# vdBerg93/cl-rrt

Hardware: AMD Instinct MI355X
Metric: nodes expanded/sec (200-obstacle scene) (higher is better)
Workload: dtype f64

## Files before the change

### cl-rrt_amd/csrc/clrrt_capi.hip

```cpp
#include <hip/hip_runtime.h>
#include <math.h>

#include <algorithm>
#include <climits>
#include <array>
#include <chrono>
#include <cmath>
#include <cstdio>
#include <cstdlib>
#include <cstring>
#include <deque>
#include <functional>
#include <optional>
#include <string>
#include <vector>

#include "../../include/clrrt.h"
#include "clrrt_dev.hpp"
#include "clrrt_internal.hpp"

static const int kWalkMaxOver = 2048, kWalkMaxChunks = 64;

using namespace clrrt;

// ... 146 lines not shown
  hipStream_t side2 = nullptr;
  hipStream_t mst = nullptr;
  int nn_delta_walk = 1;
  int nn_delta_verify = 0;
  WalkBufs nnw_d{};
  WalkBufs nnw_r{};
  struct {
    int64_t n = -1, first = 0, count = 0;
    double ox, oy, x0, y0, x1, y1;
    float delta;
    int kind, hscale;
  } nnr_built;
  int* pm_ids = nullptr;
  float* pm_keys = nullptr;
  int* pm_counts = nullptr;
  int64_t pm_cap = 0;
  int* d_bad = nullptr;
  float* vpk = nullptr;
  int* vpi = nullptr;
  float* vseed = nullptr;
  int nn_delta_early = 1;
  int nn_lane_order = 1;
  int* nn_order = nullptr;
  float* wseed[3] = {nullptr, nullptr, nullptr};
  hipEvent_t ev_wm[3] = {nullptr, nullptr, nullptr};
  hipEvent_t ev_lagw[3] = {nullptr, nullptr, nullptr};
  int stream_prio = 1;
  int walk_cu_reserve = 0;
  hipEvent_t ev_lag[3] = {nullptr, nullptr, nullptr};
  int stream_prio_applied = 0;
  bool side_prio_set = false;
  std::vector<clrrt_sample> pf_next, pf_samples;
  int pf_state = 0;
  struct {
    int T = 0;
    bool active = false;
    int R = 0;
    int T_alloc = 0, n_steps_alloc = 0;
    int64_t vcap = 0;
    RollRes* res = nullptr;
    RollRes* res_gb = nullptr;
    int* cand = nullptr;
    int* ncand = nullptr;
    clrrt_sample* samp = nullptr;
    int* best = nullptr;
    int* dlist[2] = {nullptr, nullptr};
    int cur_dl = 0, nd = 0;
    int nd_eval = -1;
    int* gv = nullptr;
    uint8_t* pend = nullptr;
    void* sel_tmp = nullptr;
    size_t sel_bytes = 0;
    int* d_cnt = nullptr;
    void* carry[2] = {nullptr, nullptr};
    int cur_c = 0, ncarry = 0, carry_cap = 0;
    int64_t round = 0;
    int slot = 0;
    int64_t deferred_total = 0;
  } def;
  struct {
    int rank = 0, world = 1;
    void* dev_local = nullptr;
    int cap_local = 0;
    clrrt_exchange_fn fn = nullptr;
    void* user = nullptr;
    double max_ms = 0;
    int64_t nd_global = 0;
    int64_t rows_stop = 0;
    int last_nb = 0;
    clrrt_node* xbuf = nullptr;
    uint32_t* xkey = nullptr;
    void* xtmp = nullptr;
    size_t xtmp_bytes = 0;
    int64_t xcap = 0;
    unsigned long long* d_goal = nullptr;
    bool poison_seen = false;
    bool fn_failed = false;
    bool hook_world1 = false;
  } sh;
  int fail_at_round = 0;
  int fail_after_exchange = 0;
  bool debug_sync = false;
  unsigned long long* dbg_host = nullptr;
  bool iter_log = false;
  std::vector<int64_t> round_sizes;
  std::vector<clrrt_iteration> iters;
  std::vector<SampleOut> iter_tmp;
  clrrt_sample* h_samples = nullptr;
  int64_t* h_totals = nullptr;
  int* h_int = nullptr;
  int64_t last_eval_rows = 0;
  int64_t last_goal_nodes = 0;
  clrrt_counters counters{};
  int64_t nn_bf_keys = 0, nn_samples = 0;
  int64_t nn_super_bounds = 0;
  bool timing = false;
  static constexpr int kKtClasses = 6;
  double kt_ms[kKtClasses] = {};
  int64_t kt_n[kKtClasses] = {};
  std::vector<hipEvent_t> ev_pool;
  std::vector<std::pair<int, std::pair<hipEvent_t, hipEvent_t>>> ev_pending;
};

static void pf_reset(clrrt_ctx* c);
static int flush_replays(clrrt_ctx* c);
static int append_nodes(clrrt_ctx* c, const clrrt_node* dev_nodes, int n);
static int watchdog_check(clrrt_ctx* c);
static void defer_roll_args(clrrt_ctx* c, RollArgs& a, bool capped);
static int commit_round(clrrt_ctx* c, int nn, double elapsed_ms, int* n_app);
static int ensure_slots(clrrt_ctx* c);

static int fail(clrrt_ctx* c, int code, const std::string& msg) {
  if (c) c->err = msg;
  return code;
}
#define HIPC(c, call)                                                                          \
  do {                                                                                         \
    hipError_t e_ = (call);                                                                    \
    if (e_ != hipSuccess)                                                                      \
      return fail((c), CLRRT_EHIP, std::string(#call) + ": " + hipGetErrorString(e_));        \
  } while (0)

template <typename T>
static hipError_t dalloc(T** p, size_t count) {
  *p = nullptr;
  if (count == 0) count = 1;
  return hipMalloc((void**)p, count * sizeof(T));
}

static hipEvent_t ev_get(clrrt_ctx* c) {
  if (!c->ev_pool.empty()) {
    hipEvent_t e = c->ev_pool.back();
    c->ev_pool.pop_back();
    return e;
  }
  hipEvent_t e;
  if (hipEventCreate(&e) != hipSuccess) return nullptr;
  return e;
}

struct KTimer {
  clrrt_ctx* c;
  int which;
  hipEvent_t a = nullptr, b = nullptr;
  hipStream_t s;
  KTimer(clrrt_ctx* c_, int w, hipStream_t s_ = nullptr) : c(c_), which(w), s(s_ ? s_ : c_->stream) {
    if (!c->timing) return;
    a = ev_get(c);
    b = ev_get(c);
    if (a) hipEventRecord(a, s);
  }
  ~KTimer() {
    if (!c->timing || !a || !b) return;
    hipEventRecord(b, s);
    c->ev_pending.push_back({which, {a, b}});
  }
};

static void drain_timers(clrrt_ctx* c) {
  for (auto& pe : c->ev_pending) {
    float ms = 0;
    hipEventSynchronize(pe.second.second);
    if (hipEventElapsedTime(&ms, pe.second.first, pe.second.second) == hipSuccess) {
      c->kt_ms[pe.first] += ms;
      c->kt_n[pe.first] += 1;
    }
// ... 149 lines not shown
static void free_all(clrrt_ctx* c) {
  if (c->side) hipStreamSynchronize(c->side);
  void* ptrs[] = {c->tree, c->nn, c->arena, c->obs, c->d_samples, c->pk, c->pi, c->cand, c->ckey, c->ncand,
                  c->ctie, c->sort_scratch, c->res_spec, c->regnodes, c->res_gb, c->gbnodes, c->so, c->first_conflict,
                  c->out_nodes, c->jobs, c->slots, c->rep_buf, c->totals, c->work_ctr, c->grid_buf,
                  c->nn_seed, c->d_bbox, c->roll_q, c->roll_best, c->roll_perm, c->roll_pflag,
                  c->goal_recs, c->bp_path, c->path_nodes, c->path_rows, c->ri_int, c->ri_off, c->ri_cost,
                  c->ri_terms, c->nnw.keys, c->nnw.keys2, c->nnw.vals, c->nnw.vals2, c->nnw.tmp, c->nnw.P, c->nnw.Q,
                  c->nnw.CE, c->nnw.ID, c->nnw.tiles, c->nnw.supers, c->nnw.sorder, c->nnw.HEAD, c->nnw.ovf_n, c->nnw.ovf, c->nnw.pk, c->nnw.pi, c->nnw_alt.keys, c->nnw_alt.keys2, c->nnw_alt.vals, c->nnw_alt.vals2, c->nnw_alt.tmp, c->nnw_alt.P, c->nnw_alt.Q, c->nnw_alt.CE, c->nnw_alt.ID, c->nnw_alt.tiles, c->nnw_alt.supers, c->nnw_alt.sorder, c->nnw_alt.HEAD, c->nnw_alt.ovf_n, c->nnw_alt.ovf, c->nnw_alt.pk, c->nnw_alt.pi, c->nnw.skeys, c->nnw.sids, c->nnw_alt.skeys, c->nnw_alt.sids, c->cmp.packed, c->cmp.scanned,
                  c->cmp.tmp, c->d_samples2, c->cand2, c->ckey2, c->ncand2, c->ctie2, c->d_samples3, c->cand3, c->ckey3,
                  c->ncand3, c->ctie3, c->nnw3.keys, c->nnw3.keys2, c->nnw3.vals, c->nnw3.vals2, c->nnw3.tmp, c->nnw3.P,
                  c->nnw3.Q, c->nnw3.CE, c->nnw3.ID, c->nnw3.tiles, c->nnw3.supers, c->nnw3.sorder, c->nnw3.HEAD,
                  c->nnw3.ovf_n, c->nnw3.ovf, c->nnw3.pk, c->nnw3.pi, c->nnw3.skeys, c->nnw3.sids,
                  c->nnw.trun, c->nnw_alt.trun, c->nnw3.trun, c->nnw.wctr, c->nnw_alt.wctr, c->nnw3.wctr};
  for (void* p : ptrs)
    if (p) hipFree(p);
  void* sptrs[] = {c->sh.xbuf, c->sh.xkey, c->sh.xtmp, c->sh.d_goal, c->fix_n, c->fix_ids, c->fix_jobs, c->fix_res, c->fix_adj,
                   c->fix_xrec, c->fix_xi, c->fix_xcand, c->fix_xkey, c->fix_xn};
  for (void* p : sptrs)
    if (p) hipFree(p);
  void* dptrs[] = {c->def.res, c->def.res_gb, c->def.cand, c->def.ncand, c->def.samp, c->def.best, c->def.dlist[0],
                   c->def.dlist[1], c->def.gv, c->def.pend, c->def.sel_tmp, c->def.d_cnt, c->def.carry[0],
                   c->def.carry[1]};
  for (void* p : dptrs)
    if (p) hipFree(p);
  if (c->h_samples) hipHostFree(c->h_samples);
  if (c->h_samples2) hipHostFree(c->h_samples2);
  if (c->h_samples3) hipHostFree(c->h_samples3);
  if (c->side2) hipStreamSynchronize(c->side2);
  if (c->side2) hipStreamDestroy(c->side2);
  for (auto e : c->ev_lag)
    if (e) hipEventDestroy(e);
  for (auto e : c->ev_lagw)
    if (e) hipEventDestroy(e);
  if (c->mst) hipStreamSynchronize(c->mst);
  if (c->mst) hipStreamDestroy(c->mst);
  for (int q = 0; q < 3; q++) {
    if (c->wseed[q]) hipFree(c->wseed[q]);
    if (q == 0 && c->nn_order) hipFree(c->nn_order);
    if (c->ev_wm[q]) hipEventDestroy(c->ev_wm[q]);
  }
  {
    WalkBufs& d = c->nnw_d;
    void* wd[] = {d.keys, d.vals, d.tmp, d.P, d.Q, d.CE, d.ID, d.HEAD, d.trun, d.tiles, d.supers, d.skeys, d.sids,
                  c->vpk, c->vpi, c->vseed};
    for (void* p : wd)
      if (p) hipFree(p);
  }
  {
    WalkBufs& r = c->nnw_r;
    void* wr[] = {r.keys, r.keys2, r.vals, r.vals2, r.tmp, r.P, r.Q, r.CE, r.ID, r.tiles, r.supers, r.sorder, r.HEAD,
                  r.ovf_n, r.ovf, r.pk, r.pi, r.skeys, r.sids, r.trun, r.wctr, c->pm_ids, c->pm_keys, c->pm_counts,
                  c->d_bad};
    for (void* p : wr)
      if (p) hipFree(p);
  }
  if (c->side) hipStreamSynchronize(c->side);
  if (c->ev_tree) hipEventDestroy(c->ev_tree);
  if (c->ev_walk) hipEventDestroy(c->ev_walk);
  if (c->ev_commit) hipEventDestroy(c->ev_commit);
  if (c->side) hipStreamDestroy(c->side);
  if (c->roll_st) hipStreamDestroy(c->roll_st);
  if (c->ev_rs0) hipEventDestroy(c->ev_rs0);
  if (c->ev_rs1) hipEventDestroy(c->ev_rs1);
  if (c->h_totals) hipHostFree(c->h_totals);
  if (c->h_int) hipHostFree(c->h_int);
  if (c->h_bbox) hipHostFree(c->h_bbox);
  if (c->dbg_host) hipHostFree(c->dbg_host);
  for (auto& pe : c->ev_pending) { hipEventDestroy(pe.second.first); hipEventDestroy(pe.second.second); }
  for (auto e : c->ev_pool) hipEventDestroy(e);
  if (c->own_stream && c->stream) hipStreamDestroy(c->stream);
}

int clrrt_create(const clrrt_params* p, const clrrt_capacity* cap, int device, clrrt_ctx** out) {
  if (!p || !out) return CLRRT_EINVAL;
  *out = nullptr;
  int ndev = 0;
  if (hipGetDeviceCount(&ndev) != hipSuccess || ndev <= 0) return CLRRT_EHIP;
  if (device < 0 || device >= ndev) return CLRRT_EINVAL;
  clrrt_ctx* c = new clrrt_ctx();
  c->device = device;
  c->params = *p;
  c->debug_sync = getenv("CLRRT_DEBUG_SYNC") != nullptr;
  clrrt_capacity dc;
  dc.max_nodes = 1 << 20;
  dc.max_rows = 1 << 24;
  dc.max_batch = 4096;
  dc.max_obstacles = 4096;
  c->cap = cap ? *cap : dc;
  if (c->cap.max_nodes < 2 || c->cap.max_rows < 2 || c->cap.max_batch < 1 || c->cap.max_obstacles < 0) {
    delete c;
    return CLRRT_EINVAL;
  }
  derive(c->params, c->dp, 0);
  int rc = CLRRT_OK;
  auto chk = [&](hipError_t e) {
    if (e != hipSuccess && rc == CLRRT_OK) { rc = CLRRT_EHIP; c->err = hipGetErrorString(e); }
  };
  chk(hipSetDevice(device));
  chk(hipStreamCreateWithFlags(&c->stream, hipStreamNonBlocking));
  c->own_stream = true;
  const int64_t B = c->cap.max_batch;
  chk(dalloc(&c->tree, c->cap.max_nodes));
  chk(dalloc(&c->nn, c->cap.max_nodes));
  chk(dalloc(&c->arena, (size_t)c->cap.max_rows * 10));
  chk(dalloc(&c->obs, std::max<int64_t>(1, c->cap.max_obstacles)));
  chk(dalloc(&c->d_samples, B));
  c->partial_cap = std::max<int64_t>(B * 16, 4096) * NN_K;
  chk(dalloc(&c->pk, c->partial_cap));
  chk(dalloc(&c->pi, c->partial_cap));
  chk(dalloc(&c->cand, B * CAND_K));
  chk(dalloc(&c->ckey, B * CAND_K));
  chk(dalloc(&c->ncand, B));
  chk(dalloc(&c->ctie, B));
  chk(dalloc(&c->d_samples2, B));
  chk(dalloc(&c->cand2, B * CAND_K));
  chk(dalloc(&c->ckey2, B * CAND_K));
  chk(dalloc(&c->ncand2, B));
  chk(dalloc(&c->ctie2, B));
  chk(hipStreamCreateWithFlags(&c->side, hipStreamNonBlocking));
  chk(hipEventCreateWithFlags(&c->ev_tree, hipEventDisableTiming));
  chk(hipEventCreateWithFlags(&c->ev_walk, hipEventDisableTiming));
  chk(hipEventCreateWithFlags(&c->ev_commit, hipEventDisableTiming));
  chk(dalloc(&c->res_spec, B * CAND_K));
  chk(dalloc(&c->regnodes, B));
  chk(dalloc(&c->res_gb, B * CAND_K));
  c->slot_rows = 0;
  chk(hipMalloc(&c->rep_buf, replay_bytes() * (size_t)2 * B));
  chk(dalloc(&c->gbnodes, B));
  chk(dalloc(&c->so, B));
  chk(dalloc(&c->first_conflict, 1));
  chk(dalloc(&c->out_nodes, 2 * B));
  chk(dalloc(&c->jobs, 2 * B));
  chk(dalloc(&c->totals, 8));
  chk(dalloc(&c->cmp.packed, B));
  chk(dalloc(&c->cmp.scanned, B));
  c->cmp.tmp_bytes = compact_scan_bytes((int)B);
  chk(hipMalloc(&c->cmp.tmp, std::max<size_t>(c->cmp.tmp_bytes, 256)));
  chk(dalloc(&c->nn_seed, B));
  chk(dalloc(&c->roll_q, 1));
  chk(dalloc(&c->roll_best, B));
  chk(dalloc(&c->roll_perm, (int64_t)B * CAND_K));
  chk(dalloc(&c->roll_pflag, (int64_t)roll_order_ints((int)(B * CAND_K))));
  {
    int ncu = 0;
    if (hipDeviceGetAttribute(&ncu, hipDeviceAttributeMultiprocessorCount, device) == hipSuccess && ncu > 0)
      c->n_cu = ncu;
  }
  chk(dalloc(&c->d_bbox, 4));
  chk(hipHostMalloc((void**)&c->h_bbox, sizeof(double) * 4, hipHostMallocDefault));
  chk(dalloc(&c->work_ctr, 64));
  if (rc == CLRRT_OK) chk(hipMemset(c->work_ctr, 0, 64 * sizeof(unsigned long long)));
  chk(hipHostMalloc((void**)&c->h_samples, sizeof(clrrt_sample) * B, hipHostMallocDefault));
  chk(hipHostMalloc((void**)&c->h_samples2, sizeof(clrrt_sample) * B, hipHostMallocDefault));
  chk(hipHostMalloc((void**)&c->h_totals, sizeof(int64_t) * 8, hipHostMallocDefault));
  chk(hipHostMalloc((void**)&c->h_int, sizeof(int) * 4, hipHostMallocDefault));
  if (rc != CLRRT_OK) {
    fprintf(stderr, "clrrt_create: %s\n", c->err.c_str());
    free_all(c);
    delete c;
    return rc;
  }
  *out = c;
  return CLRRT_OK;
}

// ... 1217 lines not shown
    if (rc != CLRRT_OK) return rc;
  }
  if (pre_roll) {
    int rc = pre_roll();
    if (rc != CLRRT_OK) return rc;
  }
  if (during_roll) HIPC(c, hipEventRecord(c->ev_tree, st));
  hipStream_t rst = st;
  if (c->roll_st) {
    rst = c->roll_st;
    HIPC(c, hipEventRecord(c->ev_rs0, st));
    HIPC(c, hipStreamWaitEvent(rst, c->ev_rs0, 0));
  }
  const bool persistent = c->roll_persistent && c->dp.n_steps_max > 0;
  const bool deferred = persistent && c->rows_deferred;
  if (!deferred) {
    int rc = flush_replays(c);
    if (rc == CLRRT_OK) rc = ensure_slots(c);
    if (rc != CLRRT_OK) return rc;
  }
  const bool defer = c->def.active && !exact && persistent && deferred;
  if (defer) {
    auto& d = c->def;
    d.slot = (int)(d.round % d.R);
    const int64_t B = c->cap.max_batch;
    HIPC(c, hipMemcpyAsync(d.cand + (int64_t)d.slot * B * CAND_K, c->cand, sizeof(int) * n * CAND_K,
                           hipMemcpyDeviceToDevice, st));
    HIPC(c, hipMemcpyAsync(d.ncand + (int64_t)d.slot * B, c->ncand, sizeof(int) * n, hipMemcpyDeviceToDevice, st));
    HIPC(c, hipMemcpyAsync(d.samp + (int64_t)d.slot * B, c->d_samples, sizeof(clrrt_sample) * n,
                           hipMemcpyDeviceToDevice, st));
    if (d.nd + (int64_t)n > d.vcap) return fail(c, CLRRT_ECAPACITY, "deferred samples exceed the commit buffers");
    if (rst != st) {
      HIPC(c, hipEventRecord(c->ev_rs0, st));
      HIPC(c, hipStreamWaitEvent(rst, c->ev_rs0, 0));
    }
  }
  {
    KTimer kt(c, 1, rst);
    RollArgs a = roll_args(c, n * CAND_K);
    a.res = c->res_spec;
    a.res_gb = c->res_gb;
    if (defer) defer_roll_args(c, a, true);
    a.slots = deferred ? nullptr : c->slots;
    a.slot_rows = c->slot_rows;
    a.slot_jobs = (int)(c->cap.max_batch * CAND_K);
    if (deferred) {
      a.rep = c->rep_buf;
      a.nrep = c->rep_n;
    }
    const int64_t nt = c->n_nodes;
    const int eighths = nt < 300000 ? 7 : nt < 700000 ? 5 : nt < 1100000 ? 4 : 2;
    const int blocks = c->roll_blocks > 0 ? std::min(c->roll_blocks, 4 * c->n_cu)
                       : c->cu_split > 0  ? std::max(1, (c->cu_split * c->n_cu) / 8)
                                          : std::max(1, (eighths * c->n_cu) / 8);
    a.coop_enable = c->roll_coop;
    a.lanes_per_wave = c->roll_lanes > 0 ? c->roll_lanes : c->roll_spread ? 0 : 64;
    if (c->roll_priority) {
      a.perm = c->roll_perm;
      a.pflag = c->roll_pflag;
      a.order_verify = c->roll_order_verify;
    }
    unsigned long long*& dbg_host = c->dbg_host;
    if (c->debug_sync) {
      if (!dbg_host) HIPC(c, hipHostMalloc((void**)&dbg_host, sizeof(unsigned long long) * 8 * 4096, hipHostMallocMapped));
      memset(dbg_host, 0, sizeof(unsigned long long) * 8 * 4096);
      HIPC(c, hipHostGetDevicePointer((void**)&a.dbg, dbg_host, 0));
      HIPC(c, hipStreamSynchronize(rst));
      fprintf(stderr, "[dbg] pre-rollout work done (n %d, nrep %d, ncarry %d)\n", n, a.nrep, a.ncarry);
    }
    if (persistent && defer) {
      FillInts f;
      f.add(a.ncarry_out, 1, 0);
      f.add(c->roll_q, 1, 0);
      f.add(c->def.best + a.sbase, n, 0x7f7f7f7f);
      f.add(c->def.d_cnt + 2, 1, 0);
      f.add((int*)c->totals, 16, 0);
      HIPC(c, launch_fill_ints(rst, f));
      c->totals_zeroed = true;
      HIPC(c, launch_rollout_persistent(rst, a, n, c->roll_q, c->def.best, blocks, true));
    } else if (persistent)
      HIPC(c, launch_rollout_persistent(rst, a, n, c->roll_q, defer ? c->def.best : c->roll_best, blocks));
    else
      HIPC(c, launch_rollout(rst, SRC_SPEC, a));
    if (c->debug_sync) {
      const auto t0 = std::chrono::steady_clock::now();
      while (hipStreamQuery(rst) == hipErrorNotReady) {
        if (std::chrono::duration<double>(std::chrono::steady_clock::now() - t0).count() > 10.0) {
          fprintf(stderr, "[dbg] rollout kernel not done after 10 s; waves (iterations, busy, parked, qdone|first "
                          "busy lane, j|pass, steps|chain, wp|N, t):\n");
          unsigned long long tmax = 0;
          for (int w = 0; w < 4096; w++) tmax = std::max(tmax, dbg_host[w * 8 + 7]);
          int shown = 0;
          for (int w = 0; w < 4096 && shown < 40; w++) {
            const unsigned long long* d = dbg_host + w * 8;
            if (d[7] == 0 || tmax - d[7] < 100000000ull) continue;
            if (d[1] == 0 && d[2] == 0 && (d[3] >> 32)) continue;
            fprintf(stderr, "  wave %d: it %llu busy %016llx parked %016llx qdone %llu lane %d j %d pass %d steps %d "
                            "chain %d wp %d N %d age %.3f s\n", w, d[0], d[1], d[2], d[3] >> 32, (int)(uint32_t)d[3],
                    (int)(d[4] >> 32), (int)(uint32_t)d[4], (int)(d[5] >> 32), (int)(uint32_t)d[5], (int)(d[6] >> 32),
                    (int)(uint32_t)d[6], (double)(tmax - d[7]) * 1e-8);
            shown++;
          }
          int alive = 0;
          for (int w = 0; w < 4096; w++) alive += dbg_host[w * 8 + 7] != 0 && tmax - dbg_host[w * 8 + 7] < 100000000ull;
          fprintf(stderr, "  waves still beating: %d\n", alive);
          abort();
        }
      }
      fprintf(stderr, "[dbg] rollout kernel done: %s\n", hipGetErrorString(hipStreamQuery(rst)));
    }
    if (deferred) c->rep_n = 0;
    c->eval_deferred = deferred;
  }
  if (c->roll_st) {
    HIPC(c, hipEventRecord(c->ev_rs1, rst));
    HIPC(c, hipStreamWaitEvent(st, c->ev_rs1, 0));
  }
  if (during_roll) {
    int rc = during_roll();
    if (rc != CLRRT_OK) return rc;
  }
  SelArgs s;
  memset(&s, 0, sizeof(s));
  s.p = c->dp; s.tree = c->tree; s.cand = c->cand; s.ckey = c->ckey; s.ncand = c->ncand; s.res = c->res_spec;
  s.res_gb = c->res_gb; s.regnodes = c->regnodes; s.gbnodes = c->gbnodes; s.so = c->so; s.B = n;
  if (defer) {
    auto& d = c->def;
    s.cand = d.cand; s.ncand = d.ncand; s.res = d.res; s.res_gb = d.res_gb;
    s.ckey = nullptr;
    s.view = d.dlist[d.cur_dl];
    s.nd = d.nd;
    s.sbase = d.slot * (int)c->cap.max_batch;
    s.gv = d.gv;
    s.pend = d.pend;
    s.new_pend = d.d_cnt + 2;
    s.B = d.nd + n;
  }
  c->def.nd_eval = defer ? c->def.nd : -1;
  {
    KTimer kt(c, 2);
    HIPC(c, launch_select(st, s));
  }
  int L = n;
  if (exact && n > 1 && c->exact_fixup) {
    int rc = exact_fixups(c, n, &L);
    if (rc != CLRRT_OK) return rc;
  } else if (exact && n > 1) {
    c->h_int[0] = n;
    HIPC(c, hipMemcpyAsync(c->first_conflict, c->h_int, sizeof(int), hipMemcpyHostToDevice, st));
    {
      KTimer kt(c, 2);
      HIPC(c, launch_conflict(st, c->dp, n, c->d_samples, c->regnodes, c->gbnodes, c->so, c->ctie,
                              c->first_conflict));
    }
    HIPC(c, hipMemcpyAsync(c->h_int + 1, c->first_conflict, sizeof(int), hipMemcpyDeviceToHost, st));
    HIPC(c, hipStreamSynchronize(st));
    L = std::max(1, std::min(n, c->h_int[1]));
  }
  *L_out = L;
  return CLRRT_OK;
}

static int compact_and_copy(clrrt_ctx* c, int L, int* n_out, bool merge_bbox) {
  hipStream_t st = c->stream;
  auto& d = c->def;
  const bool defer = d.nd_eval >= 0;
  const int V = defer ? d.nd_eval + L : L;
  {
    KTimer kt(c, 2);
    const bool tag = defer && c->sh.fn;
    HIPC(c, launch_compact(st, V, c->d_samples, c->cand, c->regnodes, c->gbnodes, c->so, c->n_rows, c->rank,
                           c->out_nodes, c->jobs, c->totals, c->cmp, tag ? d.slot : 0, tag ? d.R : 0,
                           (int)c->cap.max_batch, c->totals_zeroed));
    c->totals_zeroed = false;
    if (merge_bbox) HIPC(c, launch_bbox(st, c->out_nodes, c->totals, 0, c->d_bbox));
    if (defer) HIPC(c, launch_defer_select(st, d.gv, d.pend, V, d.dlist[1 - d.cur_dl], d.d_cnt, d.sel_tmp, d.sel_bytes));
  }
  HIPC(c, hipMemcpyAsync(c->h_totals, c->totals, sizeof(int64_t) * 8, hipMemcpyDeviceToHost, st));
  if (merge_bbox) HIPC(c, hipMemcpyAsync(c->h_bbox, c->d_bbox, sizeof(double) * 4, hipMemcpyDeviceToHost, st));
  if (defer) {
    HIPC(c, hipMemcpyAsync(c->h_int, d.d_cnt, sizeof(int) * 2, hipMemcpyDeviceToHost, st));
    HIPC(c, hipMemcpyAsync(c->h_int + 3, d.d_cnt + 2, sizeof(int), hipMemcpyDeviceToHost, st));
    HIPC(c, hipMemcpyAsync(c->h_int + 2, (const char*)(c->work_ctr + 62), sizeof(int), hipMemcpyDeviceToHost, st));
  }
  HIPC(c, hipStreamSynchronize(st));
  {
    const int rw = watchdog_check(c);
    if (rw != CLRRT_OK) return rw;
  }
  if (c->iter_log && !defer && L > 0) {
    c->iter_tmp.resize(L);
    HIPC(c, hipMemcpy(c->iter_tmp.data(), c->so, sizeof(SampleOut) * L, hipMemcpyDeviceToHost));
    for (int j = 0; j < L; j++) {
      const SampleOut& o = c->iter_tmp[j];
      clrrt_iteration r;
      r.nodes = (o.k >= 0) + (o.k >= 0 && o.gb_ok);
      r.sim_count = o.steps; r.fail_collision = o.f_col; r.fail_acclimit = o.f_acc; r.fail_iterlimit = o.f_it;
      r.rollouts = o.rollouts;
      c->iters.push_back(r);
    }
  }
  if (merge_bbox) bbox_add(c, c->h_bbox[0], c->h_bbox[1], c->h_bbox[2], c->h_bbox[3]);
  if (defer) {
    if (c->h_int[2] != 0 || c->h_int[1] > d.carry_cap)
      return fail(c, CLRRT_ECAPACITY, "suspended rollouts exceed the carry buffer (raise defer_steps)");
    if (L > 0) d.deferred_total += c->h_int[3];
    d.cur_dl ^= 1;
    d.nd = c->h_int[0];
    d.cur_c ^= 1;
    d.ncarry = c->h_int[1];
    d.round++;
    d.nd_eval = -1;
  }
  int64_t nn = c->h_totals[0], nr = c->h_totals[1];
  if (c->n_rows + nr > c->cap.max_rows) return fail(c, CLRRT_ECAPACITY, "trajectory arena full");
  if (c->fail_at_round > 0 && --c->fail_at_round == 0)
    return fail(c, CLRRT_ECAPACITY, "injected failure (option fail_at_round)");
  c->counters.sim_count += c->h_totals[2];
  c->counters.fail_collision += c->h_totals[3];
  c->counters.fail_acclimit += c->h_totals[4];
  c->counters.fail_iterlimit += c->h_totals[5];
  c->counters.rollouts += c->h_totals[6];
  c->last_goal_nodes = c->h_totals[7];
  if (c->eval_deferred) {
    if (c->rep_n > 0) {
      int rc = flush_replays(c);
      if (rc != CLRRT_OK) return rc;
    }
    KTimer kt(c, 2);
    if (defer)
      HIPC(c, launch_replay_gather(st, c->jobs, c->out_nodes, (int)nn, c->tree, d.cand, d.samp, d.res, c->rep_buf));
    else
      HIPC(c, launch_replay_gather(st, c->jobs, c->out_nodes, (int)nn, c->tree, c->cand, c->d_samples, c->res_spec,
                                   c->rep_buf));
    c->rep_n = (int)nn;
  } else {
    KTimer kt(c, 2);
    HIPC(c, launch_copy_rows(st, c->jobs, c->out_nodes, (int)nn, c->slots, c->slot_rows,
                             (int)(c->cap.max_batch * CAND_K), c->arena));
  }
  c->n_rows += nr;
  c->last_eval_rows = nr;
  *n_out = (int)nn;
  return CLRRT_OK;
}

static int ensure_defer(clrrt_ctx* c) {
  auto& d = c->def;
  const int64_t B = c->cap.max_batch;
  const int n = std::max(1, c->dp.n_steps_max);
  const int R = (int)((2LL * n + d.T - 1) / d.T) + 2;
  if (c->sh.fn && R > 256)
    return fail(c, CLRRT_EINVAL, "defer_steps too small for sharded rounds (more than 256 rounds in flight)");
  if (!d.res || d.R < R) {
    HIPC(c, hipStreamSynchronize(c->stream));
    for (void* p : {(void*)d.res, (void*)d.res_gb, (void*)d.cand, (void*)d.ncand, (void*)d.samp, (void*)d.best})
      if (p) HIPC(c, hipFree(p));
    d.res = nullptr; d.res_gb = nullptr; d.cand = nullptr; d.ncand = nullptr; d.samp = nullptr; d.best = nullptr;
    d.R = 0;
    HIPC(c, dalloc(&d.res, (size_t)R * B * CAND_K));
    HIPC(c, dalloc(&d.res_gb, (size_t)R * B * CAND_K));
    HIPC(c, dalloc(&d.cand, (size_t)R * B * CAND_K));
    HIPC(c, dalloc(&d.ncand, (size_t)R * B));
    HIPC(c, dalloc(&d.samp, (size_t)R * B));
    HIPC(c, dalloc(&d.best, (size_t)R * B));
    d.R = R;
  }
// ... 575 lines not shown
  if (c->stream_prio_applied == want || c->cu_split > 0) return CLRRT_OK;
  int lo = 0, hi = 0;
  HIPC(c, hipDeviceGetStreamPriorityRange(&lo, &hi));
  const int p_hi = c->stream_prio ? hi : 0, p_lo = c->stream_prio ? lo : 0;
  HIPC(c, hipDeviceSynchronize());
  auto remake = [&](hipStream_t& st, int pr) -> int {
    if (st) HIPC(c, hipStreamDestroy(st));
    HIPC(c, hipStreamCreateWithPriority(&st, hipStreamNonBlocking, pr));
    return CLRRT_OK;
  };
  int rc;
  if (c->walk_cu_reserve > 0) {
    const int nw = (c->n_cu + 31) / 32;
    std::vector<uint32_t> ms(nw, 0u);
    for (int i = 0; i < c->n_cu; i++)
      if ((i % 8) >= c->walk_cu_reserve) ms[i / 32] |= 1u << (i % 32);
    for (hipStream_t* st : {&c->side, &c->side2}) {
      if (*st) HIPC(c, hipStreamDestroy(*st));
      HIPC(c, hipExtStreamCreateWithCUMask(st, (uint32_t)nw, ms.data()));
    }
    if ((rc = remake(c->mst, p_hi)) != CLRRT_OK) return rc;
  } else if ((!c->side_prio_set && (rc = remake(c->side, p_lo)) != CLRRT_OK) ||
             (rc = remake(c->side2, p_lo)) != CLRRT_OK || (rc = remake(c->mst, p_hi)) != CLRRT_OK) {
    return rc;
  }
  if (c->own_stream && (rc = remake(c->stream, p_hi)) != CLRRT_OK) return rc;
  c->stream_prio_applied = want;
  return CLRRT_OK;
}

static int expand_lag2(clrrt_ctx* c, clrrt_rng* rng, int64_t n_iters, double budget_ms, int32_t batch,
                       clrrt_stats* out) {
  int rc = lag_alloc(c);
  if (rc == CLRRT_OK && c->nn_delta_walk) rc = alloc_walk_delta(c);
  if (rc == CLRRT_OK) rc = apply_stream_prio(c);
  if (rc == CLRRT_OK) rc = defer_begin(c, true);
  if (rc != CLRRT_OK) return rc;
  clrrt_stats st{};
  const auto t0 = std::chrono::steady_clock::now();
  clrrt_rng work = *rng, committed = *rng;
  std::deque<clrrt_sample> pending;
  const int cur = batch;
  const bool sharded = c->sh.fn != nullptr;
  c->sh.max_ms = 0;
  c->sh.nd_global = 0;
  c->sh.rows_stop = 0;
  shard_expansion_begin(c);
  if (sharded && (rc = shard_goal_reset(c)) != CLRRT_OK) return rc;
  const int64_t nodes_before = c->n_nodes;
  hipStream_t sides[2] = {c->side, c->side2};
  WalkBufs* W[3] = {&c->nnw, &c->nnw_alt, &c->nnw3};
  int64_t built_n[3] = {-1, -1, -1};
  double built_f[3][7] = {};
  LagSlot A, B;
  A.d = c->d_samples2; A.h = c->h_samples2; A.cand = c->cand2; A.ckey = c->ckey2; A.ncand = c->ncand2;
  A.ctie = c->ctie2; A.ev = c->ev_lag[0]; A.evw = c->ev_lagw[0];
  B.d = c->d_samples3; B.h = c->h_samples3; B.cand = c->cand3; B.ckey = c->ckey3; B.ncand = c->ncand3;
  B.ctie = c->ctie3; B.ev = c->ev_lag[1]; B.evw = c->ev_lagw[1];
  A.wseed = c->wseed[0]; A.evm = c->ev_wm[0];
  B.wseed = c->wseed[1]; B.evm = c->ev_wm[1];
  float* cur_wseed = c->wseed[2];
  hipEvent_t cur_evm = c->ev_wm[2];
  const bool early = c->nn_delta_early != 0;
  hipEvent_t cur_ev = c->ev_lag[2];
  hipEvent_t cur_evw = c->ev_lagw[2];
  const int64_t delta_walk_min = 32;
  const bool delta_walk = c->nn_delta_walk != 0;
  struct RoleGuard {
    std::function<void()> f;
    ~RoleGuard() { f(); }
  } role_guard{[&]() {
    c->d_samples2 = A.d; c->h_samples2 = A.h; c->cand2 = A.cand; c->ckey2 = A.ckey; c->ncand2 = A.ncand; c->ctie2 = A.ctie;
    c->d_samples3 = B.d; c->h_samples3 = B.h; c->cand3 = B.cand; c->ckey3 = B.ckey; c->ncand3 = B.ncand; c->ctie3 = B.ctie;
    c->ev_lag[0] = A.ev; c->ev_lag[1] = B.ev; c->ev_lag[2] = cur_ev;
    c->ev_lagw[0] = A.evw; c->ev_lagw[1] = B.evw; c->ev_lagw[2] = cur_evw;
    c->nnw_built.n = -1;
    c->nnw.sorted_n = -1;
    c->nnw_alt.sorted_n = -1;
    c->nnw3.sorted_n = -1;
  }};
  bool have_cur = false;
  int cur_stream = 0;
  double last_round_ms = 0;
  auto frame_of = [](const NnSetup& su, double* f) {
    f[0] = su.fr.ox; f[1] = su.fr.oy; f[2] = su.fr.delta; f[3] = su.x0; f[4] = su.y0; f[5] = su.x1; f[6] = su.y1;
  };
  auto build = [&](int k, const NnSetup& su) -> int {
    double f[7];
    frame_of(su, f);
    if (built_n[k] == c->n_nodes && std::equal(f, f + 7, built_f[k])) return CLRRT_OK;
    int r2 = ensure_walk_set(c, *W[k]);
    if (r2 != CLRRT_OK) return r2;
    const WalkBufs* prev = nullptr;
    for (int q = 1; q <= 2 && !prev; q++) {
      const WalkBufs* w = W[(k + 3 - q) % 3];
      if (w->P && w->sorted_n > 0) prev = w;
    }
    KTimer kt(c, 0, c->stream);
    HIPC(c, launch_nn_walk_build(c->stream, c->nn, (int)c->n_nodes, su.fr, su.x0, su.y0, su.x1, su.y1, *W[k], prev));
    built_n[k] = c->n_nodes;
    std::copy(f, f + 7, built_f[k]);
    return CLRRT_OK;
  };
  auto walk = [&](LagSlot& sl, int n, int k, const NnSetup& su, int si) -> int {
    hipStream_t s = sides[si];
    int r2 = ensure_walk_set(c, *W[k]);
    if (r2 != CLRRT_OK) return r2;
    c->nn_bf_keys += (int64_t)n * c->n_nodes;
    c->nn_samples += n;
    HIPC(c, hipStreamWaitEvent(s, c->ev_tree, 0));
    HIPC(c, hipMemcpyAsync(sl.d, sl.h, sizeof(clrrt_sample) * n, hipMemcpyHostToDevice, s));
    c->nn_super_bounds += (int64_t)n * walk_super_count(c->n_nodes);
    {
      KTimer kt(c, 0, s), kt3(c, 3, s);
      W[k]->seed_out = early ? sl.wseed : nullptr;
      W[k]->ev_main = early ? sl.evm : nullptr;
      const hipError_t ew = launch_nn_walk_search(s, sl.d, n, c->nn, (int)c->n_nodes, c->dp, su.fr, su.x0, su.y0, su.x1,
                                                  su.y1, *W[k], sl.cand, sl.ckey, sl.ncand, sl.ctie, c->work_ctr + 18,
                                                  c->nnw_stateless);
      W[k]->seed_out = nullptr;
      W[k]->ev_main = nullptr;
      HIPC(c, ew);
    }
    HIPC(c, hipEventRecord(sl.evw, s));
    sl.n = n;
    sl.tree_n = c->n_nodes;
    sl.stream = si;
    return CLRRT_OK;
  };
  auto draw_to = [&](int64_t want) {
    while ((int64_t)pending.size() < want) {
      clrrt_sample smp;
      clrrt_draw_samples(&c->params, &work, 1, &smp);
      pending.push_back(smp);
    }
  };
  for (int64_t k = 0; rc == CLRRT_OK; k++) {
    const auto tr0 = std::chrono::steady_clock::now();
    if (n_iters > 0 && st.iterations >= n_iters) break;
    const double ms0 = std::chrono::duration<double, std::milli>(tr0 - t0).count();
    if (n_iters == 0 && !((sharded ? c->sh.max_ms : ms0) < budget_ms)) break;
    const int64_t left = n_iters > 0 ? n_iters - st.iterations : INT64_MAX;
    const int64_t gb = std::min<int64_t>(cur, left);
    int64_t f0 = 0;
    int nb = (int)gb;
    if (sharded) shard_slice(c, gb, &f0, &nb);
    c->sh.last_nb = nb;
    const int64_t nc = gb + (sharded ? c->sh.nd_global : (int64_t)c->def.nd);
    if (c->n_nodes + 2 * nc > c->cap.max_nodes ||
        (sharded ? c->sh.rows_stop > 0 : c->n_rows + 2 * nc * (c->dp.n_steps_max + 1) > c->cap.max_rows)) {
      if (n_iters > 0) { rc = fail(c, CLRRT_ECAPACITY, "tree capacity exhausted"); break; }
      st.capacity_stop = 1;
      break;
    }
    const int wk = (int)(k % 3);
    const NnSetup su = nn_setup(c);
    const bool serve = c->n_nodes >= c->nnw_min_nodes && su.region_ok;
    int64_t gA = 0, gB = 0, fA = 0, fB = 0;
    int nA = 0, nB = 0;
    if (serve) {
      const bool more = n_iters > 0 || ms0 + 2.0 * last_round_ms < budget_ms;
      if (A.n == 0 && (n_iters > 0 || ms0 + last_round_ms < budget_ms)) gA = std::max<int64_t>(0, std::min<int64_t>(cur, left - gb));
      const int64_t gA_eff = A.n > 0 ? A.g : gA;
      if (more && gA_eff > 0) gB = std::max<int64_t>(0, std::min<int64_t>(cur, left - gb - gA_eff));
      nA = (int)gA;
      nB = (int)gB;
      if (sharded) {
        shard_slice(c, gA, &fA, &nA);
        shard_slice(c, gB, &fB, &nB);
      }
    }
    const int64_t gA_all = A.n > 0 ? A.g : gA;
    draw_to(gb + gA_all + gB);
    if (have_cur) {
      KTimer kt(c, 4);
      HIPC(c, hipStreamWaitEvent(c->stream, cur_ev, 0));
    } else {
      for (int j = 0; j < nb; j++) c->h_samples[j] = pending[f0 + j];
      HIPC(c, hipMemcpyAsync(c->d_samples, c->h_samples, sizeof(clrrt_sample) * nb, hipMemcpyHostToDevice, c->stream));
      if (serve) {
        HIPC(c, hipStreamSynchronize(c->side));
        HIPC(c, hipStreamSynchronize(c->side2));
        HIPC(c, hipStreamSynchronize(c->mst));
        if ((rc = build(wk, su)) != CLRRT_OK) break;
        c->nn_bf_keys += (int64_t)nb * c->n_nodes;
        c->nn_samples += nb;
        c->nn_super_bounds += (int64_t)nb * walk_super_count(c->n_nodes);
        KTimer kt(c, 0), kt3(c, 3);
        HIPC(c, launch_nn_walk_search(c->stream, c->d_samples, nb, c->nn, (int)c->n_nodes, c->dp, su.fr, su.x0, su.y0,
                                      su.x1, su.y1, *W[wk], c->cand, c->ckey, c->ncand, c->ctie, c->work_ctr + 18,
                                      c->nnw_stateless));
      } else if ((rc = run_nn(c, nb, nullptr)) != CLRRT_OK) {
        break;
      }
    }
    if (serve && (nA > 0 || nB > 0) && (rc = build(wk, su)) != CLRRT_OK) break;
    auto ahead = [&]() -> int {
      if (nA > 0) {
        for (int j = 0; j < nA; j++) A.h[j] = pending[gb + fA + j];
        const int r2 = walk(A, nA, wk, su, cur_stream);
        if (r2 != CLRRT_OK) return r2;
        A.g = gA;
      }
      if (nB > 0) {
        for (int j = 0; j < nB; j++) B.h[j] = pending[gb + gA_all + fB + j];
        const int r2 = walk(B, nB, wk, su, nA > 0 ? A.stream : 1 - A.stream);
        if (r2 != CLRRT_OK) return r2;
        B.g = gB;
      }
      return CLRRT_OK;
    };
    int L = nb, nn = 0, n_app = 0;
    if ((rc = eval_samples(c, nb, false, &L, true, (nA > 0 || nB > 0) ? std::function<int()>(ahead) : nullptr,
                           nullptr)) != CLRRT_OK)
      break;
    if ((rc = compact_and_copy(c, L, &nn, true)) != CLRRT_OK) break;
    const double ms_commit = std::chrono::duration<double, std::milli>(std::chrono::steady_clock::now() - t0).count();
    if ((rc = commit_round(c, nn, ms_commit, &n_app)) != CLRRT_OK) break;
    if (A.n > 0) {
      HIPC(c, hipEventRecord(c->ev_commit, c->stream));
      hipStream_t s = c->mst;
      HIPC(c, hipStreamWaitEvent(s, c->ev_commit, 0));
      HIPC(c, hipStreamWaitEvent(s, early ? A.evm : A.evw, 0));
      const int64_t first = A.tree_n, cnt = c->n_nodes - A.tree_n;
      const NnSetup su2 = nn_setup(c);
      const bool dwalk = delta_walk && su2.region_ok && c->n_nodes >= c->nnw_min_nodes && cnt >= delta_walk_min &&
                         cnt <= c->nnw_d.cap_nodes;
      const int max_chunks = (int)std::max<int64_t>(1, c->partial_cap / ((int64_t)A.n * NN_K));
      int nch = 0, id0 = (int)first;
      if (cnt > 0) c->nn_bf_keys += (int64_t)A.n * cnt;
      if (cnt > 0 && dwalk) {
        KTimer kt(c, 0, s);
        float* seed = early ? A.wseed : c->nn_seed;
        const bool verify = c->nn_delta_verify && c->vseed;
        HIPC(c, launch_nn_delta_walk(s, A.d, A.n, c->nn, (int)first, (int)cnt, c->dp, su2.fr, su2.x0, su2.y0, su2.x1,
                                     su2.y1, c->nnw_d, c->pk, c->pi, A.ckey, A.ncand, seed, early,
                                     verify ? c->work_ctr + 40 : nullptr));
        nch = 1;
        id0 = 0;
        if (verify) {
          int vch = 0;
          HIPC(c, hipMemcpyAsync(c->vseed, seed, sizeof(float) * A.n, hipMemcpyDeviceToDevice, s));
          HIPC(c, launch_nn_delta_partial(s, A.d, A.n, c->nn, (int)first, (int)cnt, c->dp, su2.fr, c->vpk, c->vpi,
                                          max_chunks, nullptr, nullptr, c->vseed, true, nullptr, &vch, c->work_ctr + 52));
          HIPC(c, launch_nn_delta_compare(s, A.n, vch, (int)first, c->vpk, c->vpi, c->pk, c->pi, c->work_ctr + 38));
        }
      } else if (cnt > 0 && early) {
        KTimer kt(c, 0, s);
        HIPC(c, launch_nn_delta_partial(s, A.d, A.n, c->nn, (int)first, (int)cnt, c->dp, su2.fr, c->pk, c->pi,
                                        max_chunks, nullptr, nullptr, A.wseed, true,
                                        c->nn_lane_order ? c->nn_order : nullptr, &nch));
      } else if (cnt > 0) {
        KTimer kt(c, 0, s);
        HIPC(c, launch_nn_delta(s, A.d, A.n, c->nn, (int)first, (int)cnt, c->dp, su2.fr, c->pk, c->pi, max_chunks,
                                A.cand, A.ckey, A.ncand, A.ctie, c->nn_seed));
      }
      if (early) HIPC(c, hipStreamWaitEvent(s, A.evw, 0));
      if (nch > 0) {
        KTimer kt(c, 0, s);
        HIPC(c, launch_nn_delta_merge(s, A.n, nch, c->dp, c->pk, c->pi, id0, A.cand, A.ckey, A.ncand, A.ctie));
      }
      HIPC(c, hipEventRecord(A.ev, s));
    }
    {
      const NnSetup sn = nn_setup(c);
      if (B.n > 0 && c->n_nodes >= c->nnw_min_nodes && sn.region_ok && (rc = build((int)((k + 1) % 3), sn)) != CLRRT_OK)
        break;
    }
    for (int64_t j = 0; j < gb; j++) {
      pending.pop_front();
      for (int q = 0; q < 3; q++) clrrt_rng_next(&committed);
    }
    st.iterations += gb;
    st.goal_nodes_added += c->last_goal_nodes;
    st.speculated += gb;
    st.rounds++;
    {
      LagSlot old;
      old.d = c->d_samples; old.h = c->h_samples; old.cand = c->cand; old.ckey = c->ckey; old.ncand = c->ncand;
      old.ctie = c->ctie; old.ev = cur_ev; old.evw = cur_evw; old.stream = cur_stream;
      old.wseed = cur_wseed; old.evm = cur_evm;
      have_cur = A.n > 0;
      c->d_samples = A.d; c->h_samples = A.h; c->cand = A.cand; c->ckey = A.ckey; c->ncand = A.ncand; c->ctie = A.ctie;
      cur_ev = A.ev;
      cur_evw = A.evw;
      cur_stream = A.stream;
      cur_wseed = A.wseed; cur_evm = A.evm;
      A = B;
      B = old;
      B.n = 0;
      B.stream = 1 - A.stream;
    }
    last_round_ms = std::chrono::duration<double, std::milli>(std::chrono::steady_clock::now() - tr0).count();
  }
  if (rc == CLRRT_OK) rc = defer_drain(c, &st.goal_nodes_added);
  st.deferred = c->def.deferred_total;
  if (rc == CLRRT_OK) rc = flush_replays(c);
  if (rc == CLRRT_OK && sharded) rc = shard_goal_count(c, &st.goal_nodes_added);
  rc = shard_expansion_end(c, rc);
  c->def.active = false;
  for (hipStream_t s : {c->side, c->side2, c->mst, c->stream}) {
    const hipError_t e = hipStreamSynchronize(s);
    if (e != hipSuccess && rc == CLRRT_OK) rc = fail(c, CLRRT_EHIP, std::string("hipStreamSynchronize: ") + hipGetErrorString(e));
  }
  st.nodes_added = c->n_nodes - nodes_before;
  st.elapsed_ms = std::chrono::duration<double, std::milli>(std::chrono::steady_clock::now() - t0).count();
  *rng = committed;
  if (out) *out = st;
  return rc;
}

int clrrt_expand(clrrt_ctx* c, clrrt_rng* rng, int64_t n_iters, double budget_ms, int32_t mode, int32_t batch,
                 clrrt_stats* out) {
  if (!c || !rng || n_iters < 0 || (mode != CLRRT_MODE_EXACT && mode != CLRRT_MODE_BATCH)) return CLRRT_EINVAL;
  pf_reset(c);
  if (n_iters == 0 && !(budget_ms > 0)) return CLRRT_EINVAL;
  if (c->n_nodes <= 0) return fail(c, CLRRT_ESTATE, "tree not initialised");
  c->round_sizes.clear();
  const bool sharded = c->sh.fn != nullptr;
  if (sharded && mode != CLRRT_MODE_BATCH) return fail(c, CLRRT_EINVAL, "sharded expansion runs BATCH rounds only");
  HIPC(c, hipSetDevice(c->device));
  const int64_t bmax = (int64_t)c->cap.max_batch * c->sh.world;
  batch = (int32_t)std::max<int64_t>(1, std::min<int64_t>(batch > 0 ? batch : bmax, bmax));
  if (sharded && batch < c->sh.world) return fail(c, CLRRT_EINVAL, "fewer samples per round than ranks");
  const int lag = c->nn_lag ? c->nn_lag
                  : (n_iters == 0 ? budget_ms >= 1000.0 : n_iters >= 64 * (int64_t)batch) ? 2 : 1;
  if (mode == CLRRT_MODE_BATCH && c->nn_pipeline && lag == 2) return expand_lag2(c, rng, n_iters, budget_ms, batch, out);
  clrrt_stats st{};
  auto t0 = std::chrono::steady_clock::now();
  clrrt_rng work = *rng;
  clrrt_rng committed = *rng;
  std::deque<clrrt_sample> pending;
  const bool exact = mode == CLRRT_MODE_EXACT;
  int cur = exact ? std::min(batch, std::max(16, c->exact_min_width)) : batch;
  int64_t nodes_before = c->n_nodes;
  int rc = defer_begin(c, !exact);
  c->sh.max_ms = 0;
  c->sh.nd_global = 0;
  c->sh.rows_stop = 0;
  shard_expansion_begin(c);
  if (rc == CLRRT_OK && sharded) rc = shard_goal_reset(c);
  bool have_next = false;
  double last_round_ms = 0;
  auto draw_to = [&](int64_t want) {
    while ((int64_t)pending.size() < want) {
      clrrt_sample smp;
      clrrt_draw_samples(&c->params, &work, 1, &smp);
      pending.push_back(smp);
    }
  };
  for (; rc == CLRRT_OK;) {
    const auto tr0 = std::chrono::steady_clock::now();
    if (n_iters > 0 && st.iterations >= n_iters) break;
    if (n_iters == 0) {
      double ms = std::chrono::duration<double, std::milli>(std::chrono::steady_clock::now() - t0).count();
      if (!((sharded ? c->sh.max_ms : ms) < budget_ms)) break;
    }
    int64_t gb = cur;
    if (n_iters > 0) gb = std::min<int64_t>(gb, n_iters - st.iterations);
    int64_t f0 = 0;
    int nb = (int)gb;
    if (sharded) shard_slice(c, gb, &f0, &nb);
    c->sh.last_nb = nb;
    const int64_t nc = gb + (sharded ? c->sh.nd_global : (int64_t)c->def.nd);
    if (c->n_nodes + 2 * nc > c->cap.max_nodes ||
        (sharded ? c->sh.rows_stop > 0 : c->n_rows + 2 * nc * (c->dp.n_steps_max + 1) > c->cap.max_rows)) {
      if (n_iters > 0) { rc = fail(c, CLRRT_ECAPACITY, "tree capacity exhausted"); break; }
      st.capacity_stop = 1;
      break;
    }
    draw_to(gb);
    if (!have_next) {
      for (int j = 0; j < nb; j++) c->h_samples[j] = pending[f0 + j];
      HIPC(c, hipMemcpyAsync(c->d_samples, c->h_samples, sizeof(clrrt_sample) * nb, hipMemcpyHostToDevice, c->stream));
    }
    int64_t gb2 = 0, f2 = 0;
    int nb2 = 0;
    NnSetup su{};
    if (!exact && c->nn_pipeline) {
      gb2 = cur;
      if (n_iters > 0) gb2 = std::max<int64_t>(0, std::min<int64_t>(gb2, n_iters - st.iterations - gb));
      if (n_iters == 0) {
        double ms = std::chrono::duration<double, std::milli>(std::chrono::steady_clock::now() - t0).count();
        if (!(ms + last_round_ms < budget_ms)) gb2 = 0;
      }
      nb2 = (int)gb2;
      if (sharded) shard_slice(c, gb2, &f2, &nb2);
      if (nb2 > 0) {
        su = nn_setup(c);
        if (!walk_serves(c, su)) nb2 = 0;
      }
    }
    auto prefetch = [&]() -> int {
      draw_to(gb + gb2);
      for (int j = 0; j < nb2; j++) c->h_samples2[j] = pending[gb + f2 + j];
      return launch_side_walk(c, nb2, su);
    };
    int L = nb, nn = 0, n_app = 0;
    auto build = [&]() -> int { return pre_roll_build(c, su); };
    if ((rc = eval_samples(c, nb, exact, &L, have_next, nb2 > 0 ? std::function<int()>(prefetch) : nullptr,
                           nb2 > 0 ? std::function<int()>(build) : nullptr)) != CLRRT_OK)
      break;
    if (!exact) {
      int64_t want = gb + (int64_t)cur;
      if (n_iters > 0) want = std::min<int64_t>(want, n_iters - st.iterations);
      draw_to(want);
    }
    if ((rc = compact_and_copy(c, L, &nn, true)) != CLRRT_OK) break;
    const int64_t first_new = c->n_nodes;
    const double ms_commit = std::chrono::duration<double, std::milli>(std::chrono::steady_clock::now() - t0).count();
    if ((rc = commit_round(c, nn, ms_commit, &n_app)) != CLRRT_OK) break;
    have_next = false;
    if (nb2 > 0) {
      if ((rc = side_delta_launch(c, nb2, first_new, n_app)) != CLRRT_OK) break;
      if (c->nnw_double && (rc = next_round_build(c)) != CLRRT_OK) break;
      if ((rc = side_lists_join(c)) != CLRRT_OK) break;
      have_next = true;
    }
    const int64_t used = exact ? L : gb;
    for (int64_t j = 0; j < used; j++) {
      pending.pop_front();
      for (int k = 0; k < 3; k++) clrrt_rng_next(&committed);
    }
    st.iterations += used;
    st.goal_nodes_added += c->last_goal_nodes;
    st.speculated += exact ? nb : gb;
    st.rounds++;
    if (exact) cur = std::max(c->exact_min_width, std::min(batch, L == nb ? 2 * nb : 2 * L));
    last_round_ms = std::chrono::duration<double, std::milli>(std::chrono::steady_clock::now() - tr0).count();
  }
  if (rc == CLRRT_OK) rc = defer_drain(c, &st.goal_nodes_added);
  st.deferred = c->def.deferred_total;
// ... 349 lines not shown
```

Before: 1.482 million.

## Overlap host RNG retirement and sample drawing with device work; add host-gap probe

```diff
diff --git a/cl-rrt_amd/csrc/clrrt_capi.hip b/cl-rrt_amd/csrc/clrrt_capi.hip
--- a/cl-rrt_amd/csrc/clrrt_capi.hip
+++ b/cl-rrt_amd/csrc/clrrt_capi.hip
@@ -252,6 +252,8 @@
   int fail_after_exchange = 0;
   bool debug_sync = false;
   unsigned long long* dbg_host = nullptr;
+  bool host_gap = false;
+  std::chrono::steady_clock::time_point t_roll_launch{};
   bool iter_log = false;
   std::vector<int64_t> round_sizes;
   std::vector<clrrt_iteration> iters;
@@ -567,6 +569,7 @@
   c->device = device;
   c->params = *p;
   c->debug_sync = getenv("CLRRT_DEBUG_SYNC") != nullptr;
+  c->host_gap = getenv("CLRRT_HOST_GAP") != nullptr;
   clrrt_capacity dc;
   dc.max_nodes = 1 << 20;
   dc.max_rows = 1 << 24;
@@ -1950,6 +1953,7 @@
       HIPC(c, launch_rollout_persistent(rst, a, n, c->roll_q, defer ? c->def.best : c->roll_best, blocks));
     else
       HIPC(c, launch_rollout(rst, SRC_SPEC, a));
+    if (c->host_gap) c->t_roll_launch = std::chrono::steady_clock::now();
     if (c->debug_sync) {
       const auto t0 = std::chrono::steady_clock::now();
       while (hipStreamQuery(rst) == hipErrorNotReady) {
@@ -2029,7 +2033,8 @@
   return CLRRT_OK;
 }
 
-static int compact_and_copy(clrrt_ctx* c, int L, int* n_out, bool merge_bbox) {
+static int compact_and_copy(clrrt_ctx* c, int L, int* n_out, bool merge_bbox,
+                            const std::function<void()>& before_sync = nullptr) {
   hipStream_t st = c->stream;
   auto& d = c->def;
   const bool defer = d.nd_eval >= 0;
@@ -2051,6 +2056,7 @@
     HIPC(c, hipMemcpyAsync(c->h_int + 3, d.d_cnt + 2, sizeof(int), hipMemcpyDeviceToHost, st));
     HIPC(c, hipMemcpyAsync(c->h_int + 2, (const char*)(c->work_ctr + 62), sizeof(int), hipMemcpyDeviceToHost, st));
   }
+  if (before_sync) before_sync();
   HIPC(c, hipStreamSynchronize(st));
   {
     const int rw = watchdog_check(c);
@@ -2792,6 +2798,15 @@
   bool have_cur = false;
   int cur_stream = 0;
   double last_round_ms = 0;
+  struct HostGap {
+    double us[2][6] = {};
+    int64_t n[2] = {};
+    std::chrono::steady_clock::time_point t[4];
+    bool open = false;
+  } hg;
+  auto hg_us = [](std::chrono::steady_clock::time_point a, std::chrono::steady_clock::time_point b) {
+    return std::chrono::duration<double, std::micro>(b - a).count();
+  };
   auto frame_of = [](const NnSetup& su, double* f) {
     f[0] = su.fr.ox; f[1] = su.fr.oy; f[2] = su.fr.delta; f[3] = su.x0; f[4] = su.y0; f[5] = su.x1; f[6] = su.y1;
   };
@@ -2838,12 +2853,13 @@
     sl.stream = si;
     return CLRRT_OK;
   };
+  std::vector<clrrt_sample> drawn;
   auto draw_to = [&](int64_t want) {
-    while ((int64_t)pending.size() < want) {
-      clrrt_sample smp;
-      clrrt_draw_samples(&c->params, &work, 1, &smp);
-      pending.push_back(smp);
-    }
+    const int64_t n = want - (int64_t)pending.size();
+    if (n <= 0) return;
+    drawn.resize((size_t)n);
+    clrrt_draw_samples(&c->params, &work, (int32_t)n, drawn.data());
+    pending.insert(pending.end(), drawn.begin(), drawn.end());
   };
   for (int64_t k = 0; rc == CLRRT_OK; k++) {
     const auto tr0 = std::chrono::steady_clock::now();
@@ -2882,6 +2898,7 @@
     }
     const int64_t gA_all = A.n > 0 ? A.g : gA;
     draw_to(gb + gA_all + gB);
+    if (c->host_gap) hg.t[3] = std::chrono::steady_clock::now();
     if (have_cur) {
       KTimer kt(c, 4);
       HIPC(c, hipStreamWaitEvent(c->stream, cur_ev, 0));
@@ -2924,7 +2941,30 @@
     if ((rc = eval_samples(c, nb, false, &L, true, (nA > 0 || nB > 0) ? std::function<int()>(ahead) : nullptr,
                            nullptr)) != CLRRT_OK)
       break;
-    if ((rc = compact_and_copy(c, L, &nn, true)) != CLRRT_OK) break;
+    if (c->host_gap && hg.open) {
+      const double d[5] = {hg_us(hg.t[0], hg.t[1]), hg_us(hg.t[1], hg.t[2]), hg_us(hg.t[2], hg.t[3]),
+                           hg_us(hg.t[3], c->t_roll_launch), hg_us(hg.t[0], c->t_roll_launch)};
+      for (int w = 0; w < (c->n_nodes >= 1100000 ? 2 : 1); w++) {
+        for (int q = 0; q < 5; q++) hg.us[w][q] += d[q];
+        hg.n[w]++;
+      }
+    }
+    clrrt_rng committed_next = committed;
+    bool retire_ready = false;
+    auto under_roll = [&]() {
+      const auto tu0 = std::chrono::steady_clock::now();
+      for (int64_t j = 0; j < 3 * gb; j++) clrrt_rng_next(&committed_next);
+      retire_ready = true;
+      const int64_t rest = n_iters > 0 ? left - gb : INT64_MAX;
+      draw_to(gb + std::min<int64_t>(3 * (int64_t)cur, rest));
+      if (c->host_gap) {
+        const double d = hg_us(tu0, std::chrono::steady_clock::now());
+        hg.us[0][5] += d;
+        if (c->n_nodes >= 1100000) hg.us[1][5] += d;
+      }
+    };
+    if ((rc = compact_and_copy(c, L, &nn, true, under_roll)) != CLRRT_OK) break;
+    if (c->host_gap) hg.t[0] = std::chrono::steady_clock::now();
     const double ms_commit = std::chrono::duration<double, std::milli>(std::chrono::steady_clock::now() - t0).count();
     if ((rc = commit_round(c, nn, ms_commit, &n_app)) != CLRRT_OK) break;
     if (A.n > 0) {
@@ -2977,9 +3017,14 @@
       if (B.n > 0 && c->n_nodes >= c->nnw_min_nodes && sn.region_ok && (rc = build((int)((k + 1) % 3), sn)) != CLRRT_OK)
         break;
     }
-    for (int64_t j = 0; j < gb; j++) {
-      pending.pop_front();
-      for (int q = 0; q < 3; q++) clrrt_rng_next(&committed);
+    if (c->host_gap) hg.t[1] = std::chrono::steady_clock::now();
+    if (!retire_ready)
+      for (int64_t j = 0; j < 3 * gb; j++) clrrt_rng_next(&committed_next);
+    committed = committed_next;
+    pending.erase(pending.begin(), pending.begin() + gb);
+    if (c->host_gap) {
+      hg.t[2] = std::chrono::steady_clock::now();
+      hg.open = true;
     }
     st.iterations += gb;
     st.goal_nodes_added += c->last_goal_nodes;
@@ -3015,6 +3060,14 @@
   }
   st.nodes_added = c->n_nodes - nodes_before;
   st.elapsed_ms = std::chrono::duration<double, std::milli>(std::chrono::steady_clock::now() - t0).count();
+  if (c->host_gap)
+    for (int w = 0; w < 2; w++) {
+      const double m = hg.n[w] > 0 ? 1.0 / (double)hg.n[w] : 0.0;
+      fprintf(stderr, "[host_gap] %s rounds %lld batch %d: mean us sync->enqueued %.1f, ->retired %.1f, ->drawn %.1f, "
+                      "->rollout launch %.1f, whole path %.1f; host work under the rollout kernel %.1f\n",
+              w ? "late (>= 1.1 M nodes)" : "all", (long long)hg.n[w], cur, hg.us[w][0] * m, hg.us[w][1] * m,
+              hg.us[w][2] * m, hg.us[w][3] * m, hg.us[w][4] * m, hg.us[w][5] * m);
+    }
   *rng = committed;
   if (out) *out = st;
   return rc;
@@ -3052,12 +3105,13 @@
   if (rc == CLRRT_OK && sharded) rc = shard_goal_reset(c);
   bool have_next = false;
   double last_round_ms = 0;
+  std::vector<clrrt_sample> drawn;
   auto draw_to = [&](int64_t want) {
-    while ((int64_t)pending.size() < want) {
-      clrrt_sample smp;
-      clrrt_draw_samples(&c->params, &work, 1, &smp);
-      pending.push_back(smp);
-    }
+    const int64_t n = want - (int64_t)pending.size();
+    if (n <= 0) return;
+    drawn.resize((size_t)n);
+    clrrt_draw_samples(&c->params, &work, (int32_t)n, drawn.data());
+    pending.insert(pending.end(), drawn.begin(), drawn.end());
   };
   for (; rc == CLRRT_OK;) {
     const auto tr0 = std::chrono::steady_clock::now();
```

Result: no change. 1.488 million, median of 6 (+0.4%).
